# CrispyChillies/Image-Retrieval---Thesis-2026

Measured on AMD Instinct MI355X. Metric: queries/sec (embed+top-10) over 1M x 1024 gallery, higher is better.
Workload: dtype f32 embed (two fp16 MFMA terms); bf16 MFMA candidates + f64 re-rank

## Files before the change

image-retrieval---thesis-2026_amd/_lib.py:

```python
import ctypes
import os

_HERE = os.path.dirname(os.path.abspath(__file__))
LIB_PATH = os.environ.get("MIRX_LIB_PATH", os.path.join(_HERE, "libmirx.so"))

METRIC_IP = 0
METRIC_NEG_L2 = 1
TIER_AUTO = 0
TIER_EXACT_ONLY = 3
OPT_TIERS = 1
OPT_SAMPLE_RANK = 2
OPT_FORCE_TAU = 3
OPT_PROFILE = 4
OPT_RANK_SORT = 5
RANK_SORT_AUTO = 0
RANK_SORT_BITONIC = 1
RANK_SORT_RADIX = 2
MAX_SEARCH_K = 1024
TUNE_CONV1X1_SMALL_MAX_WG = 1
TUNE_CONV3X3_SMALL_MAX_WG = 2
TUNE_CONV1X1_RING = 3
SIMCAM_MAPS_BOTH = 0
SIMCAM_MAPS_RETRIEVED = 1
SIMATT_GROUP = 0
SIMATT_PAIRS = 1
ANOMALY_BAD_SCORE = 1
ANOMALY_BAD_NORM = 2
ANOMALY_BAD_ONE_CLASS = 4
ANOMALY_BAD_EMPTY_CLASS = 8
RESAMPLE_MAX_SIDE = 8192
RESAMPLE_MAX_TAPS = 65
RESAMPLE_MAX_OUT = 1024
RESAMPLE_MAX_BATCH = 65536
RESAMPLE_MAX_LDS = 65536
RESAMPLE_TILE_W, RESAMPLE_TILE_H = 32, 16
RESAMPLE_DESC_WORDS = 8
# ... 9 lines not shown

class SearchStats(ctypes.Structure):
    _fields_ = [(n, ctypes.c_int64) for n in
                ("nq", "tier1_answered", "exact_answered", "candidates", "reranked",
                 "overflowed", "incomplete")]

    def as_dict(self):
        return {n: int(getattr(self, n)) for n, _ in self._fields_}


_vp, _i64, _int = ctypes.c_void_p, ctypes.c_int64, ctypes.c_int
SYMBOLS = {
    "mirx_last_error": (ctypes.c_char_p, []),
    "mirx_version": (_int, []),
    "mirx_set_tuning": (_int, [_int, _i64]),
    "mirx_index_create": (_int, [_int, _int, _int, ctypes.POINTER(_vp)]),
    "mirx_index_destroy": (None, [_vp]),
    "mirx_index_add": (_int, [_vp, _vp, _i64, _vp]),
    "mirx_index_reserve": (_int, [_vp, _i64]),
    "mirx_index_size": (_i64, [_vp]),
    "mirx_index_dim": (_int, [_vp]),
    "mirx_index_set_option": (_int, [_vp, _int, _i64]),
    "mirx_index_get_rows": (_int, [_vp, _i64, _i64, _vp, _vp]),
    "mirx_index_search": (_int, [_vp, _vp, _i64, _int, _vp, _vp, _vp, _vp]),
    "mirx_index_search_f64": (_int, [_vp, _vp, _i64, _int, _vp, _vp, _vp, _vp]),
    "mirx_index_search_begin": (_int, [_vp, _vp, _i64, _int, _vp, _vp, _vp, _vp, _vp]),
    "mirx_index_search_end": (_int, [_vp]),
    "mirx_index_last_stats": (_int, [_vp, _vp, ctypes.POINTER(SearchStats)]),
    "mirx_index_last_timings": (_int, [_vp, ctypes.POINTER(ctypes.c_float)]),
    "mirx_index_rank_all": (_int, [_vp, _vp, _i64, _vp, _vp, _vp, _vp]),
# ... 35 lines not shown
    "mirx_dense_layer_fused": (_int, [_vp, _i64, _i64, _int, _vp, _vp, _vp, _vp, _vp, _vp, _vp, _i64, _int, _vp, ctypes.c_float,
                                      ctypes.c_float, ctypes.c_float, ctypes.c_float, _vp]),
    "mirx_conv3x3_direct_terms_nchw": (_int, [_vp, _vp, _vp, _i64, _int, _vp, _i64, _vp, _vp, _i64, _vp]),
    "mirx_conv3x3_direct_terms_nchw_pool": (_int, [_vp, _vp, _vp, _i64, _int, _vp, _i64, _vp, _vp, _i64, _vp, _vp, _vp, _i64, _vp]),
    "mirx_conv3x3_small_launch": (_int, [_i64, _int]),
    "mirx_conv3x3_winograd_split3_nchw": (_int, [_vp, _vp, _i64, _int, _vp, _i64, _vp]),
    "mirx_conv3x3_direct_split3_nchw": (_int, [_vp, _vp, _i64, _int, _vp, _i64, _vp]),
    "mirx_conv3x3_winograd_nchw": (_int, [_vp, _vp, _i64, _int, _vp, _i64, _vp]),
    "mirx_attention_qkv_f32": (_int, [_vp, _i64, _int, _int, _int, ctypes.c_float, _vp, _vp]),
    "mirx_attention_qkv_f32_split2h": (_int, [_vp, _i64, _int, _int, _int, ctypes.c_float, ctypes.c_float, ctypes.c_float, _vp, _vp]),
    "mirx_attention_qkv_f32_split2h_terms": (_int, [_vp, _i64, _int, _int, _int, ctypes.c_float, ctypes.c_float, ctypes.c_float,
                                                    ctypes.c_float, _vp, _vp]),
    "mirx_attention_qkv_f32_split3": (_int, [_vp, _i64, _int, _int, _int, ctypes.c_float, _vp, _vp]),
    "mirx_l2_normalize": (_int, [_vp, _i64, _int, _vp]),
    "mirx_bn_relu_gap_l2norm": (_int, [_vp, _vp, _vp, _i64, _int, _int, _int, _vp, _vp]),
    "mirx_bn_relu_nchw": (_int, [_vp, _i64, _vp, _vp, _i64, _int, _int, _vp, _vp]),
    "mirx_bn_relu_avgpool2": (_int, [_vp, _i64, _vp, _vp, _i64, _int, _int, _int, _vp, _i64, _vp]),
    "mirx_bn_relu_avgpool2_into": (_int, [_vp, _i64, _vp, _vp, _i64, _int, _int, _int, _vp, _i64, _i64, _vp]),
    "mirx_conv1x1_bn_relu": (_int, [_vp, _i64, _int, _vp, _vp, _vp, _vp, _i64, _int, _int, _int, _vp, _vp]),
    "mirx_dwconv7x7_nchw_to_nhwc": (_int, [_vp, _vp, _vp, _i64, _int, _int, _int, _vp, _vp]),
    "mirx_dwconv7x7_nhwc": (_int, [_vp, _vp, _vp, _i64, _int, _int, _int, _vp, _vp]),
    "mirx_stem_conv7_bn_relu_pool_split3": (_int, [_vp, _vp, _vp, _vp, _i64, _int, _int, _vp, _vp]),
    "mirx_stem_conv7_bn_relu_pool": (_int, [_vp, _vp, _vp, _vp, _i64, _int, _int, _vp, _vp]),
    "mirx_conv_terms": (_int, [_vp, _vp, _vp, _i64, _int, _int, _int, _int, _int, _vp, _vp, _vp, _int, ctypes.c_float,
                               ctypes.c_float, _vp, _vp, _vp, _int, _vp, _vp, _vp, _vp, _vp]),
    "mirx_nchw_to_terms": (_int, [_vp, _i64, _i64, _int, _int, _vp, _vp, _vp, _vp]),
    "mirx_gap_nhwc_l2norm": (_int, [_vp, _i64, _int, _int, _int, _vp, _vp]),
    "mirx_window_attention_split2h": (_int, [_vp, _i64, _int, _int, _int, _int, _int, _vp, _vp, _vp, _vp, ctypes.c_float, _vp]),
    "mirx_swin_postnorm": (_int, [_vp, _vp, _i64, _int, _vp, _vp, ctypes.c_float, _vp, _vp, ctypes.c_float, _vp]),
    "mirx_patch_merge_terms": (_int, [_vp, _i64, _int, _int, _int, ctypes.c_float, _vp, _vp]),
# ... 82 lines not shown
```

image-retrieval---thesis-2026_amd/csrc/k_conv1x1_h2.hip:

```cpp
#include <atomic>

#include "mirx_device.h"
#include "mirx_kernels.h"

namespace mirx {

namespace {

#ifdef MIRX_C1H2_STAMPS
__device__ unsigned long long g_c1_stamps[8192 * 8];
#define C1_STAMP(ACC)                                                 \
    {                                                                 \
        const unsigned long long now_ = __builtin_amdgcn_s_memtime(); \
        ACC += now_ - st_t;                                           \
        st_t = now_;                                                  \
    }
#else
#define C1_STAMP(ACC)
#endif

constexpr int CM = 128;
constexpr int CP = 128;
constexpr int KC = 16;
constexpr int PLANE_A = CM * KC * 2;
// ... 650 lines not shown
#pragma unroll
            for (int mi = 0; mi < 4; ++mi)
#pragma unroll
                for (int r = 0; r < 16; ++r) {
                    const int ch = mi * 32 + (r & 3) + 8 * (r >> 2) + 4 * (lane >> 5);
                    float v = fmaf(acc[mi][ni][r], TABLED ? sOsc[ep_k[ni]][ch] : sOsc[0][ch] * x_inv, sBias[ch]);
                    if (RELU_OUT) v = v < 0.f ? 0.f : v;
                    vmax = range_max(vmax, v);
                    yo[(int64_t)(co0 + ch) * yps] = v;
                }
        }
        if (out_amax) range_publish_lanes(out_amax, (int)bimg, vmax, lane);
    }
}

template <bool PROLOGUE, bool RELU_OUT, bool YTERMS, int NPT, bool TABLED, bool RING>
__global__ __launch_bounds__(256, NPT == 2 ? 2 : 3) void k_conv1x1_h2(C1H2_PARAMS) {
    if constexpr (RING) conv1x1_ring<PROLOGUE, RELU_OUT, YTERMS, TABLED>(C1H2_ARGS);
    else conv1x1_tiled<PROLOGUE, RELU_OUT, YTERMS, NPT, TABLED>(C1H2_ARGS);
}

}

#ifdef MIRX_C1H2_STAMPS
extern "C" int mirx_debug_c1_stamps(unsigned long long *out) {
    return (int)hipMemcpyFromSymbol(out, HIP_SYMBOL(g_c1_stamps), sizeof(g_c1_stamps));
}
#endif

static std::atomic<int> g_small_max_wg{128};
void set_conv1x1_small_max_wg(int v) { g_small_max_wg.store(v < 0 ? 0 : v); }
static int conv1x1_small_max_wg() { return g_small_max_wg.load(std::memory_order_relaxed); }
static std::atomic<int> g_ring{1};
void set_conv1x1_ring(int v) { g_ring.store(v ? 1 : 0); }
static bool conv1x1_ring_enabled() { return g_ring.load(std::memory_order_relaxed) != 0; }

hipError_t launch_conv1x1_h2(const float *x, int64_t xbs, int cin, const float *scale, const float *shift,
                             const uint16_t *w2, const float *oscale, const float *bias, int64_t n, int hw, int cout,
                             int relu_out, float *y, int64_t ybs, const float *in_amax, float in_ks, float in_kb,
                             float *out_amax, float y_ks, float y_kb, float *y_inv_out, int64_t xps, int64_t yps,
                             hipStream_t st) {
    if (n <= 0) return hipSuccess;
    if (cin % KC || cout % CM || !oscale) return hipErrorInvalidValue;
    const bool yterms = y_inv_out != nullptr;
    if (yterms && (cout != CM || !relu_out || !scale)) return hipErrorInvalidValue;
    if (!xps) xps = hw;
    if (!yps) yps = hw;
    if (xps < hw || yps < hw) return hipErrorInvalidValue;
    const int64_t px = n * (int64_t)hw;
    if (px >= ((int64_t)1 << 31) - 2 * CP) return hipErrorInvalidValue;
    if (yterms && px >= ((int64_t)1 << 27)) return hipErrorInvalidValue;
    const bool small_bn_ok = !scale || (cin <= 1024 && ((reinterpret_cast<uintptr_t>(scale) | reinterpret_cast<uintptr_t>(shift)) & 15) == 0);
    if (px * (cout / CM) < (int64_t)CP * conv1x1_small_max_wg() && small_bn_ok)
        return launch_conv1x1_h2_small(x, xbs, cin, scale, shift, w2, oscale, bias, n, hw, cout, relu_out, y, ybs, in_amax,
                                       in_ks, in_kb, out_amax, y_ks, y_kb, y_inv_out, xps, yps, st);
    const int npt = px >= (int64_t)2 * CP * MIRX_C1H2_MIN_WG ? MIRX_C1H2_NPT : 1;
    const bool ring = npt == 2 && conv1x1_ring_enabled() && hw % 4 == 0 && xps % 4 == 0 && xbs % 4 == 0 &&
                      (reinterpret_cast<uintptr_t>(x) & 15) == 0 && (!scale || cin <= RING_BN_MAX_CIN) &&
                      ((int64_t)((RNP - 1) / hw + 2) * xbs + (int64_t)cin * xps) * 4 < ((int64_t)1 << 31);
    const dim3 grid((unsigned)((px + CP * npt - 1) / (CP * npt)), (unsigned)(cout / CM));
    const size_t lds = ring ? (size_t)RING_BN + (scale ? (size_t)cin * 8 : 0) : 2 * (size_t)(2 * PLANE_A + npt * 2 * PLANE_B);
    unsigned *oa = reinterpret_cast<unsigned *>(out_amax);
    const bool tabled = (CP * npt - 1) / hw + 2 <= 8;
#define MIRX_H2K(P, R, T, N, RG)                                                                           \
    {                                                                                                      \
        if (tabled) MIRX_H2KT(P, R, T, N, true, RG) else MIRX_H2KT(P, R, T, N, false, RG)                  \
    }
#define MIRX_H2KT(P, R, T, N, TB, RG)                                                                      \
    {                                                                                                      \
        static std::atomic<unsigned long long> attr_devs{0};       \
        hipError_t e = set_dynamic_lds(k_conv1x1_h2<P, R, T, N, TB, RG>, RG ? RING_BN + 8 * RING_BN_MAX_CIN : 2 * (2 * PLANE_A + N * 2 * PLANE_B), &attr_devs);    \
        if (e != hipSuccess) return e;                                                                 \
        hipLaunchKernelGGL((k_conv1x1_h2<P, R, T, N, TB, RG>), grid, dim3(256), lds, st, x, xbs, cin, scale, shift, w2, oscale, \
                           bias, n, hw, cout, y, ybs, in_amax, in_ks, in_kb, oa, y_ks, y_kb, y_inv_out, xps, yps); \
    }
#define MIRX_H2C(P, R, T)                                                                                  \
    {                                                                                                      \
// ... 17 lines not shown
```

image-retrieval---thesis-2026_amd/csrc/k_prep.hip:

```cpp
#include "mirx_device.h"
#include "mirx_kernels.h"

#include <algorithm>

namespace mirx {

namespace {

__device__ inline double row_sumsq_lane_tree(const float *__restrict__ x, int dim) {
    const int lane = lane_id();
    const int nchunk = (dim + 3) >> 2;
    const bool vec = ((dim & 3) == 0) && ((reinterpret_cast<uintptr_t>(x) & 15) == 0);
    double acc = 0.0;
    for (int c = lane; c < nchunk; c += WAVE) {
        float v[4];
        if (vec) {
            const float4 t = *reinterpret_cast<const float4 *>(x + 4 * c);
            v[0] = t.x; v[1] = t.y; v[2] = t.z; v[3] = t.w;
        } else {
#pragma unroll
            for (int e = 0; e < 4; ++e) v[e] = (4 * c + e < dim) ? x[4 * c + e] : 0.0f;
        }
#pragma unroll
        for (int e = 0; e < 4; ++e) acc = fma((double)v[e], (double)v[e], acc);
// ... 55 lines not shown
}

__global__ __launch_bounds__(256) void k_l2_normalize(float *__restrict__ x, int64_t n, int dim) {
    const int64_t row = (int64_t)blockIdx.x * 4 + (threadIdx.x >> 6);
    if (row >= n) return;
    float *r = x + row * dim;
    const double ss = row_sumsq_lane_tree(r, dim);
    double nrm = sqrt(ss);
    if (nrm < 1e-12) nrm = 1e-12;
    for (int e = lane_id(); e < dim; e += WAVE) r[e] = (float)((double)r[e] / nrm);
}

constexpr int HEAD_THREADS = 1024;
__global__ __launch_bounds__(HEAD_THREADS) void k_head(const float *__restrict__ x,
                                              const float *__restrict__ scale,
                                              const float *__restrict__ shift, int c, int hw,
                                              int normalize, float *__restrict__ y) {
    extern __shared__ __attribute__((aligned(16))) float mean_s[];
    const int64_t b = blockIdx.x;
    const int wave = threadIdx.x >> 6, lane = lane_id();
    const float *xb = x + b * (int64_t)c * hw;
    const float inv = 1.0f / (float)hw;
    constexpr int UC = 8;
    for (int ch0 = wave * UC; ch0 < c; ch0 += (HEAD_THREADS / WAVE) * UC) {
        float acc[UC];
#pragma unroll
        for (int u = 0; u < UC; ++u) {
            const int ch = ch0 + u < c ? ch0 + u : c - 1;
            const float sc = scale ? scale[ch] : 1.0f, sh = shift ? shift[ch] : 0.0f;
            const float *p = xb + (int64_t)ch * hw;
            acc[u] = 0.0f;
            for (int i = lane; i < hw; i += WAVE) {
                const float t = fmaf(p[i], sc, sh);
                acc[u] += t < 0.0f ? 0.0f : t;
            }
        }
#pragma unroll
        for (int u = 0; u < UC; ++u) {
#pragma unroll
            for (int off = 32; off >= 1; off >>= 1) acc[u] += __shfl_xor(acc[u], off, 64);
            if (lane == 0 && ch0 + u < c) mean_s[ch0 + u] = acc[u] * inv;
        }
    }
    const int cpad = (c + 3) & ~3;
    double *nrm_s = reinterpret_cast<double *>(mean_s + cpad);
    for (int i = c + threadIdx.x; i < cpad; i += HEAD_THREADS) mean_s[i] = 0.0f;
    __syncthreads();
    if (normalize) {
        if (wave == 0) {
            const double ss = row_sumsq_lane_tree(mean_s, c);
            double nrm = sqrt(ss);
            if (nrm < 1e-12) nrm = 1e-12;
            if (lane == 0) *nrm_s = nrm;
        }
        __syncthreads();
        const double nrm = *nrm_s;
        for (int i = threadIdx.x; i < c; i += HEAD_THREADS) y[b * c + i] = (float)((double)mean_s[i] / nrm);
    } else {
        for (int i = threadIdx.x; i < c; i += HEAD_THREADS) y[b * c + i] = mean_s[i];
    }
}

__global__ __launch_bounds__(256) void k_bn_relu(const float *__restrict__ x, int64_t xbs,
                                                 const float *__restrict__ scale,
                                                 const float *__restrict__ shift, int c, int hw,
                                                 float *__restrict__ y) {
    const int64_t b = blockIdx.y;
    const int64_t slab = (int64_t)c * hw;
    const float *xb = x + b * xbs;
    float *yb = y + b * slab;
    const float inv_hw = 1.0f / (float)hw;
    for (int64_t e = ((int64_t)blockIdx.x * 256 + threadIdx.x) * 4; e < slab; e += (int64_t)gridDim.x * 1024) {
        const float4 v = *reinterpret_cast<const float4 *>(xb + e);
        int ch = (int)((float)e * inv_hw);
// ... 102 lines not shown

hipError_t launch_prep_queries(const float *q, int64_t nq, int64_t nq_pad, int dim, int dimp,
                               float *q32p, uint16_t *q16, float *qnorm, hipStream_t st) {
    if (nq_pad <= 0) return hipSuccess;
    hipLaunchKernelGGL(k_prep_queries, dim3((unsigned)((nq_pad + 3) / 4)), dim3(256), 0, st, q, nq,
                       nq_pad, dim, dimp, q32p, q16, qnorm);
    return hipGetLastError();
}

hipError_t launch_l2_normalize(float *x, int64_t n, int dim, hipStream_t st) {
    if (n <= 0) return hipSuccess;
    hipLaunchKernelGGL(k_l2_normalize, dim3((unsigned)((n + 3) / 4)), dim3(256), 0, st, x, n, dim);
    return hipGetLastError();
}

hipError_t launch_bn_relu_gap_l2norm(const float *x, const float *scale, const float *shift,
                                     int64_t n, int c, int hw, int normalize, float *y,
                                     hipStream_t st) {
    if (n <= 0) return hipSuccess;
    const size_t lds = (size_t)((c + 3) & ~3) * sizeof(float) + 16;
    hipLaunchKernelGGL(k_head, dim3((unsigned)n), dim3(HEAD_THREADS), lds, st, x, scale, shift, c, hw,
                       normalize, y);
    return hipGetLastError();
}

}
```

image-retrieval---thesis-2026_amd/csrc/mirx_api.hip:

```cpp
#include <algorithm>
#include <cmath>
#include <cstring>
#include <new>
#include <mutex>
#include <vector>

#include "mirx_kernels.h"

namespace mirx {

static thread_local std::string g_err;
void set_error(const std::string &msg) { g_err = msg; }
int fail(int code, const std::string &msg) {
    g_err = msg;
    return code;
}

static inline int64_t round_up(int64_t v, int64_t m) { return (v + m - 1) / m * m; }

struct DevBuf {
    void *p = nullptr;
    size_t bytes = 0;
    hipError_t ensure(size_t need) {
        if (need <= bytes) return hipSuccess;
// ... 490 lines not shown

int mirx_set_tuning(int key, int64_t value) {
    switch (key) {
        case MIRX_TUNE_CONV1X1_SMALL_MAX_WG:
            MIRX_CHECK(value >= 0 && value <= (1 << 20), "set_tuning: conv1x1 small-launch limit out of range");
            set_conv1x1_small_max_wg((int)value);
            return MIRX_OK;
        case MIRX_TUNE_CONV3X3_SMALL_MAX_WG:
            MIRX_CHECK(value >= 0 && value <= (1 << 20), "set_tuning: conv3x3 small-launch limit out of range");
            set_conv3x3_small_max_wg((int)value);
            return MIRX_OK;
        case MIRX_TUNE_CONV1X1_RING:
            MIRX_CHECK(value == 0 || value == 1, "set_tuning: conv1x1 ring switch must be 0 or 1");
            set_conv1x1_ring((int)value);
            return MIRX_OK;
        default:
            return fail(MIRX_EINVAL, "set_tuning: unknown key");
    }
}

int mirx_index_create(int dim, int metric, int device, mirx_index **out) {
    MIRX_CHECK(out, "index_create: out is null");
    *out = nullptr;
    MIRX_CHECK(dim >= 1 && round_up(dim, DIM_ALIGN) <= MAX_DIMP, "index_create: dim out of range");
    MIRX_CHECK(metric == MIRX_METRIC_IP || metric == MIRX_METRIC_NEG_L2, "index_create: unknown metric");
    int ndev = 0;
    MIRX_HIP(hipGetDeviceCount(&ndev));
    MIRX_CHECK(device >= 0 && device < ndev, "index_create: no such device");
    DeviceGuard dg(device);
    if (!dg.ok) return fail(MIRX_EHIP, "index_create: cannot select device");
    mirx_index *ix = new (std::nothrow) mirx_index();
    if (!ix) return fail(MIRX_ENOMEM, "index_create: host allocation failed");
// ... 679 lines not shown

int mirx_l2_normalize(float *x, int64_t n, int dim, void *stream) {
    MIRX_CHECK(x && n >= 0 && dim >= 1, "l2_normalize: bad argument");
    MIRX_HIP(launch_l2_normalize(x, n, dim, reinterpret_cast<hipStream_t>(stream)));
    return MIRX_OK;
}

int mirx_bn_relu_gap_l2norm(const float *x, const float *scale, const float *shift, int64_t n, int c,
                            int hw, int normalize, float *y, void *stream) {
    MIRX_CHECK(x && y && n >= 0 && c >= 1 && c <= 16384 && hw >= 1, "bn_relu_gap_l2norm: bad argument");
    MIRX_HIP(launch_bn_relu_gap_l2norm(x, scale, shift, n, c, hw, normalize, y,
                                       reinterpret_cast<hipStream_t>(stream)));
    return MIRX_OK;
}

int mirx_bn_relu_nchw(const float *x, int64_t x_batch_stride, const float *scale, const float *shift,
                      int64_t n, int c, int hw, float *y, void *stream) {
    MIRX_CHECK(x && scale && shift && y && n >= 0 && c >= 1 && hw >= 1, "bn_relu_nchw: bad argument");
    MIRX_CHECK(((int64_t)c * hw) % 4 == 0 && x_batch_stride % 4 == 0 && x_batch_stride >= (int64_t)c * hw,
               "bn_relu_nchw: c*hw and the batch stride must be multiples of 4");
    MIRX_HIP(launch_bn_relu_nchw(x, x_batch_stride, scale, shift, n, c, hw, y,
                                 reinterpret_cast<hipStream_t>(stream)));
    return MIRX_OK;
}

int mirx_bn_relu_avgpool2(const float *x, int64_t x_batch_stride, const float *scale, const float *shift,
                          int64_t n, int c, int h, int w, float *y, int64_t x_plane_stride, void *stream) {
    MIRX_CHECK(x && scale && shift && y && n >= 0 && c >= 1, "bn_relu_avgpool2: bad argument");
    MIRX_CHECK(h >= 2 && w >= 2 && h % 2 == 0 && w % 2 == 0 && x_batch_stride % 2 == 0,
               "bn_relu_avgpool2: h, w and the batch stride must be even");
// ... 343 lines not shown
```

image-retrieval---thesis-2026_amd/csrc/mirx_kernels.h:

```cpp
#pragma once
#include "mirx_common.h"

namespace mirx {

hipError_t launch_ingest(const float *src, int64_t n, int dim, int dimp, float *g32,
                         uint16_t *g16, float *gbias, unsigned *gnorm_max_bits, int metric,
                         hipStream_t st);
hipError_t launch_prep_queries(const float *q, int64_t nq, int64_t nq_pad, int dim, int dimp,
                               float *q32p, uint16_t *q16, float *qnorm, hipStream_t st);
hipError_t launch_l2_normalize(float *x, int64_t n, int dim, hipStream_t st);
hipError_t launch_bn_relu_gap_l2norm(const float *x, const float *scale, const float *shift,
                                     int64_t n, int c, int hw, int normalize, float *y,
                                     hipStream_t st);
hipError_t launch_bn_relu_nchw(const float *x, int64_t x_batch_stride, const float *scale,
                               const float *shift, int64_t n, int c, int hw, float *y, hipStream_t st);
hipError_t launch_bn_relu_avgpool2(const float *x, int64_t x_batch_stride, const float *scale,
                                   const float *shift, int64_t n, int c, int h, int w, float *y,
                                   int64_t x_plane_stride, hipStream_t st, int64_t y_batch_stride = 0);
hipError_t launch_stem(const float *x, const float *w, const float *scale, const float *shift,
                       int64_t n, int h, int wd, float *y, hipStream_t st);
hipError_t launch_stem_s3(const float *x, const uint16_t *w3, const float *scale, const float *shift, int64_t n, int h,
                          int wd, float *y, int64_t y_bs, float *out_range, hipStream_t st);

hipError_t launch_stem_h2(const float *x, const uint16_t *w2, const float *oscale, const float *scale, const float *shift,
                          int64_t n, int h, int wd, float *y, int64_t y_bs, const float *in_range, float *out_range,
                          hipStream_t st);
hipError_t launch_range_absmax(const float *x, int64_t per_image, int64_t n, float *row, hipStream_t st);
hipError_t launch_stem_h2_u8(const uint8_t *x, const float *mean, const float *stdv, const uint16_t *w2, const float *oscale,
// ... 73 lines not shown
hipError_t launch_resample(const void *blob_dev, int64_t b, int s, int out_f32, const float *mean3, const float *std3, void *out,
                           int64_t lds, hipStream_t st);

hipError_t launch_conv1x1_s3(const float *x, int64_t xbs, int cin, const float *scale, const float *shift,
                             const uint16_t *w3, const float *bias, int64_t n, int hw, int cout, int relu_out,
                             float *y, int64_t ybs, hipStream_t st);

hipError_t launch_conv1x1_h2(const float *x, int64_t xbs, int cin, const float *scale, const float *shift,
                             const uint16_t *w2, const float *oscale, const float *bias, int64_t n, int hw, int cout,
                             int relu_out, float *y, int64_t ybs, const float *in_amax, float in_ks, float in_kb,
                             float *out_amax, float y_ks, float y_kb, float *y_inv_out, int64_t xps, int64_t yps,
                             hipStream_t st);

void set_conv1x1_small_max_wg(int v);
void set_conv1x1_ring(int v);
hipError_t launch_conv1x1_h2_small(const float *x, int64_t xbs, int cin, const float *scale, const float *shift,
                                   const uint16_t *w2, const float *oscale, const float *bias, int64_t n, int hw, int cout,
                                   int relu_out, float *y, int64_t ybs, const float *in_amax, float in_ks, float in_kb,
                                   float *out_amax, float y_ks, float y_kb, float *y_inv_out, int64_t xps, int64_t yps,
                                   hipStream_t st);

hipError_t launch_linear_h2(const float *x, int64_t m, int k, const uint16_t *w2, const float *bias, int n, int act,
                            const float *res, const float *gamma, float x_scale, float out_scale, float *y,
                            int tokens_per_image, const float *xb_dev, hipStream_t st, bool rows_out = false,
                            float *sq_out = nullptr);
hipError_t launch_grn_norm_partials(const float *part, int tpi, int64_t n_img, int c, float *gx, hipStream_t st);

hipError_t launch_linear_s3(const float *x, int64_t m, int k, const uint16_t *w3, const float *bias, int n, int act,
                            const float *res, const float *gamma, float *y, int tokens_per_image, hipStream_t st);

// ... 140 lines not shown
```

include/mirx.h:

```cpp
#ifndef MIRX_H
#define MIRX_H

#include <stdint.h>

#ifdef __cplusplus
extern "C" {
#endif

#define MIRX_VERSION 305

#define MIRX_OK 0
#define MIRX_EINVAL (-1)
#define MIRX_ENOMEM (-2)
#define MIRX_EHIP (-3)
#define MIRX_ESTATE (-4)

#define MIRX_METRIC_IP 0
#define MIRX_METRIC_NEG_L2 1

#define MIRX_TIER_AUTO 0
#define MIRX_TIER_EXACT_ONLY 3

#define MIRX_OPT_TIERS 1
#define MIRX_OPT_SAMPLE_RANK 2
// ... 18 lines not shown
    int64_t nq;
    int64_t tier1_answered;
    int64_t exact_answered;
    int64_t candidates;
    int64_t reranked;
    int64_t overflowed;
    int64_t incomplete;
} mirx_search_stats;

const char *mirx_last_error(void);
int mirx_version(void);

#define MIRX_TUNE_CONV1X1_SMALL_MAX_WG 1
#define MIRX_TUNE_CONV3X3_SMALL_MAX_WG 2
#define MIRX_TUNE_CONV1X1_RING 3
int mirx_set_tuning(int key, int64_t value);

int mirx_index_create(int dim, int metric, int device, mirx_index **out);
void mirx_index_destroy(mirx_index *ix);

int mirx_index_add(mirx_index *ix, const float *rows, int64_t n, const int64_t *ids_or_null);
int mirx_index_reserve(mirx_index *ix, int64_t capacity_rows);
int64_t mirx_index_size(const mirx_index *ix);
int mirx_index_dim(const mirx_index *ix);
int mirx_index_set_option(mirx_index *ix, int option, int64_t value);

int mirx_index_get_rows(const mirx_index *ix, int64_t first, int64_t n, float *out_rows,
                        int64_t *out_ids_or_null);

int mirx_index_search(mirx_index *ix, const float *q, int64_t nq, int k,
                      const int64_t *exclude_ids_or_null, float *out_scores, int64_t *out_ids,
// ... 128 lines not shown
                                   float scale, float qk_bound, float v_bound, float *out, void *stream);
int mirx_attention_qkv_f32_split2h_terms(const float *qkv, int64_t batch, int n_tokens, int heads, int head_dim, float scale,
                                         float qk_bound, float v_bound, float out_scale, void *out_terms, void *stream);

int mirx_rank_metrics(const int64_t *ranks, int64_t nq, int64_t n, int64_t row_stride,
                      const int64_t *gallery_labels, int64_t n_labels, const int64_t *query_labels,
                      const int64_t *query_ids_or_null, int drop_self, int rel_kind,
                      double jaccard_threshold, int ap_kind, const int32_t *kappas, int nk,
                      double *out_ap, int64_t *out_cnt, int64_t *out_nrel, int64_t *out_maxpos,
                      void *stream);

int mirx_l2_normalize(float *x, int64_t n, int dim, void *stream);

int mirx_bn_relu_gap_l2norm(const float *x, const float *scale, const float *shift, int64_t n,
                            int c, int hw, int normalize, float *y, void *stream);

int mirx_bn_relu_nchw(const float *x, int64_t x_batch_stride, const float *scale, const float *shift,
                      int64_t n, int c, int hw, float *y, void *stream);

int mirx_bn_relu_avgpool2(const float *x, int64_t x_batch_stride, const float *scale,
                          const float *shift, int64_t n, int c, int h, int w, float *y, int64_t x_plane_stride,
                          void *stream);
int mirx_bn_relu_avgpool2_into(const float *x, int64_t x_batch_stride, const float *scale, const float *shift,
                               int64_t n, int c, int h, int w, float *y, int64_t y_batch_stride, int64_t x_plane_stride,
                               void *stream);

int mirx_stem_conv7_bn_relu_pool(const float *x, const float *w, const float *scale,
                                 const float *shift, int64_t n, int h, int wd, float *y,
                                 void *stream);

// ... 214 lines not shown
```

Baseline: 43070.

## Add wide 256-channel conv1x1 kernel and run-staged GAP head kernel

Adds a conv1x1 variant in which each workgroup computes 256 output channels over 128 pixels, with buffer-to-LDS DMA into a three-slot ring so each input tile is reused across twice as many channels. It is used by default for large no-BN-prologue launches. It also adds a head kernel that stages contiguous runs of small spatial planes in LDS with float4 loads before the BN-ReLU-GAP-L2 reduction, plus tuning switches and launch counters. In exchange, the wide kernel carries a larger accumulator count and more LDS per block, which may reduce occupancy.

```diff
diff --git a/image-retrieval---thesis-2026_amd/_lib.py b/image-retrieval---thesis-2026_amd/_lib.py
--- a/image-retrieval---thesis-2026_amd/_lib.py
+++ b/image-retrieval---thesis-2026_amd/_lib.py
@@ -20,6 +20,9 @@
 TUNE_CONV1X1_SMALL_MAX_WG = 1
 TUNE_CONV3X3_SMALL_MAX_WG = 2
 TUNE_CONV1X1_RING = 3
+TUNE_CONV1X1_WIDE = 4
+TUNE_HEAD_RUNS = 5
+TUNE_CONV1X1_LARGE_MIN_WG = 6
 SIMCAM_MAPS_BOTH = 0
 SIMCAM_MAPS_RETRIEVED = 1
 SIMATT_GROUP = 0
@@ -59,6 +62,7 @@
     "mirx_last_error": (ctypes.c_char_p, []),
     "mirx_version": (_int, []),
     "mirx_set_tuning": (_int, [_int, _i64]),
+    "mirx_launch_count": (_i64, [_int]),
     "mirx_index_create": (_int, [_int, _int, _int, ctypes.POINTER(_vp)]),
     "mirx_index_destroy": (None, [_vp]),
     "mirx_index_add": (_int, [_vp, _vp, _i64, _vp]),
@@ -124,6 +128,7 @@
     "mirx_attention_qkv_f32_split3": (_int, [_vp, _i64, _int, _int, _int, ctypes.c_float, _vp, _vp]),
     "mirx_l2_normalize": (_int, [_vp, _i64, _int, _vp]),
     "mirx_bn_relu_gap_l2norm": (_int, [_vp, _vp, _vp, _i64, _int, _int, _int, _vp, _vp]),
+    "mirx_bn_relu_gap_l2norm_strided": (_int, [_vp, _i64, _vp, _vp, _i64, _int, _int, _int, _vp, _vp]),
     "mirx_bn_relu_nchw": (_int, [_vp, _i64, _vp, _vp, _i64, _int, _int, _vp, _vp]),
     "mirx_bn_relu_avgpool2": (_int, [_vp, _i64, _vp, _vp, _i64, _int, _int, _int, _vp, _i64, _vp]),
     "mirx_bn_relu_avgpool2_into": (_int, [_vp, _i64, _vp, _vp, _i64, _int, _int, _int, _vp, _i64, _i64, _vp]),
diff --git a/image-retrieval---thesis-2026_amd/csrc/k_conv1x1_h2.hip b/image-retrieval---thesis-2026_amd/csrc/k_conv1x1_h2.hip
--- a/image-retrieval---thesis-2026_amd/csrc/k_conv1x1_h2.hip
+++ b/image-retrieval---thesis-2026_amd/csrc/k_conv1x1_h2.hip
@@ -688,6 +688,182 @@
     }
 }
 
+constexpr int WSLOT_W = 2 * 2 * PLANE_A;
+constexpr int WSLOT = WSLOT_W + KC * CP * 4;
+constexpr int WIDE_LDS = RSLOTS * WSLOT;
+
+template <bool RELU_OUT, bool TABLED, bool DW>
+__device__ __forceinline__ void conv1x1_wide(C1H2_PARAMS) {
+    extern __shared__ __attribute__((aligned(16))) char sm[];
+    constexpr int KIMG = 8;
+    constexpr int WCM = 2 * CM;
+    constexpr int PIECES = 4 + (DW ? 8 : 2);
+    const int wave = __builtin_amdgcn_readfirstlane(threadIdx.x >> 6), lane = threadIdx.x & 63;
+    const int tid = threadIdx.x;
+    const int64_t total = n * (int64_t)hw;
+    const int64_t p0 = (int64_t)blockIdx.x * CP;
+    const int co0 = blockIdx.y * WCM;
+    const int nk = cin / KC;
+    auto image_bound = [&](int64_t img) { return fmaf(in_ks, in_amax ? in_amax[img] : 0.f, in_kb); };
+    const unsigned img_first = (unsigned)p0 / (unsigned)hw;
+    const unsigned p_last = (unsigned)(p0 + CP - 1 < total ? p0 + CP - 1 : total - 1);
+
+    const __amdgpu_buffer_rsrc_t wrsrc = __builtin_amdgcn_make_buffer_rsrc(
+        (void *)(w2 + ((int64_t)(2 * blockIdx.y) * nk) * (2 * CM * KC)), 0, 2 * nk * (2 * CM * KC * 2), 0x00020000);
+    const int w_voff = (lane >> 1) * 32 + (((lane & 1) ^ ((lane >> 4) & 1)) << 4);
+    const __amdgpu_buffer_rsrc_t xrsrc =
+        __builtin_amdgcn_make_buffer_rsrc((void *)(x + (int64_t)img_first * xbs), 0, 0x7fffffff, 0x00020000);
+    const int xps4 = (int)xps * 4;
+    auto pixel_voff = [&](unsigned pp) {
+        if (pp >= (unsigned)total) return 0;
+        const unsigned pimg = pp / (unsigned)hw;
+        return (int)(((int64_t)(pimg - img_first) * xbs + (pp - pimg * (unsigned)hw)) * 4);
+    };
+    int x_voff[2];
+    if (DW) {
+        x_voff[0] = pixel_voff((unsigned)p0 + lane);
+        x_voff[1] = pixel_voff((unsigned)p0 + 64u + lane);
+    } else {
+        x_voff[0] = pixel_voff((unsigned)p0 + 4u * (lane & 31)) + (lane >> 5) * xps4;
+        x_voff[1] = 0;
+    }
+    auto dma = [&](int kt, int slot) {
+        char *sb = sm + slot * WSLOT;
+#pragma unroll
+        for (int i = 0; i < 4; ++i) {
+            const int piece = wave + 4 * i;
+            __builtin_amdgcn_raw_ptr_buffer_load_lds(wrsrc, LDS_PTR(sb + piece * 1024), 16, w_voff,
+                                                     ((piece >> 3) * nk + kt) * (2 * CM * KC * 2) + (piece & 7) * 1024, 0, 0);
+        }
+        if (DW) {
+#pragma unroll
+            for (int i = 0; i < 8; ++i) {
+                const int c = 4 * wave + (i >> 1), h = i & 1;
+                __builtin_amdgcn_raw_ptr_buffer_load_lds(xrsrc, LDS_PTR(sb + WSLOT_W + c * (CP * 4) + h * 256), 4, x_voff[h],
+                                                         (kt * KC + c) * xps4, 0, 0);
+            }
+        } else {
+#pragma unroll
+            for (int i = 0; i < 2; ++i) {
+                const int pc = 2 * wave + i;
+                __builtin_amdgcn_raw_ptr_buffer_load_lds(xrsrc, LDS_PTR(sb + WSLOT_W + pc * 1024), 16, x_voff[0],
+                                                         (kt * KC + 2 * pc) * xps4, 0, 0);
+            }
+        }
+    };
+
+    const float t_bias = bias ? bias[co0 + tid] : 0.f;
+    const float t_osc = oscale[co0 + tid];
+    const unsigned nimg = p_last / (unsigned)hw - img_first + 1;
+    float ib[KIMG];
+#pragma unroll
+    for (int k = 0; k < KIMG; ++k) ib[k] = TABLED && (unsigned)k < nimg ? image_bound(img_first + k) : 0.f;
+    unsigned col_img;
+    {
+        unsigned pp = (unsigned)(p0 + 32 * wave + (lane & 31));
+        if (pp >= (unsigned)total) pp = (unsigned)total - 1u;
+        col_img = pp / (unsigned)hw;
+    }
+    const float col_bound = image_bound(col_img);
+    __builtin_amdgcn_sched_barrier(0);
+    dma(0, 0);
+    if (nk > 1) dma(1, 1);
+    __builtin_amdgcn_sched_barrier(0);
+    float x_scale, ep_xinv;
+    range_scales(col_bound, x_scale, ep_xinv);
+    const int ep_k = TABLED ? (int)(col_img - img_first) : 0;
+    if (TABLED) ep_xinv = 1.f;
+
+    const int kg = lane >> 5;
+    int fa[4];
+#pragma unroll
+    for (int mi = 0; mi < 4; ++mi) {
+        const int ra_ = mi * 32 + (lane & 31);
+        fa[mi] = ra_ * 32 + ((kg ^ ((ra_ >> 3) & 1)) << 4);
+    }
+    const int fb = WSLOT_W + 8 * kg * (CP * 4) + (32 * wave + (lane & 31)) * 4;
+
+    f32x16 acc[8];
+#pragma unroll
+    for (int mi = 0; mi < 8; ++mi)
+#pragma unroll
+        for (int r = 0; r < 16; ++r) acc[mi][r] = 0.f;
+
+    int slot = 0;
+    for (int kt = 0; kt < nk; ++kt) {
+        if (kt + 1 < nk) asm volatile("s_waitcnt vmcnt(%0)" ::"n"(PIECES) : "memory");
+        else asm volatile("s_waitcnt vmcnt(0)" ::: "memory");
+        asm volatile("s_waitcnt lgkmcnt(0)\n\ts_barrier" ::: "memory");
+        if (kt + 2 < nk) dma(kt + 2, slot == 0 ? 2 : slot - 1);
+        __builtin_amdgcn_sched_barrier(0);
+        const char *sb = sm + slot * WSLOT;
+        u32x4 ph, pl;
+#pragma unroll
+        for (int j = 0; j < 4; ++j) {
+            const float v0 = *reinterpret_cast<const float *>(sb + fb + (2 * j) * (CP * 4));
+            const float v1 = *reinterpret_cast<const float *>(sb + fb + (2 * j + 1) * (CP * 4));
+            unsigned th, tl;
+            split2h_pair(v0 * x_scale, v1 * x_scale, th, tl);
+            ph[j] = th;
+            pl[j] = tl;
+        }
+        const f16x8 b0 = __builtin_bit_cast(f16x8, ph), b1 = __builtin_bit_cast(f16x8, pl);
+#pragma unroll
+        for (int mi = 0; mi < 8; ++mi) {
+            const f16x8 a0 = *reinterpret_cast<const f16x8 *>(sb + (mi >> 2) * (2 * PLANE_A) + fa[mi & 3]);
+            const f16x8 a1 = *reinterpret_cast<const f16x8 *>(sb + (mi >> 2) * (2 * PLANE_A) + fa[mi & 3] + PLANE_A);
+            f32x16 c = acc[mi];
+            c = __builtin_amdgcn_mfma_f32_32x32x16_f16(a1, b0, c, 0, 0, 0);
+            c = __builtin_amdgcn_mfma_f32_32x32x16_f16(a0, b1, c, 0, 0, 0);
+            c = __builtin_amdgcn_mfma_f32_32x32x16_f16(a0, b0, c, 0, 0, 0);
+            acc[mi] = c;
+        }
+        slot = slot == RSLOTS - 1 ? 0 : slot + 1;
+    }
+
+    float *sBias = reinterpret_cast<float *>(sm + (nk % RSLOTS) * WSLOT);
+    float(*sOsc)[WCM] = reinterpret_cast<float(*)[WCM]>(sBias + WCM);
+    sBias[tid] = t_bias;
+    sOsc[0][tid] = t_osc;
+    if (TABLED) {
+#pragma unroll
+        for (int k = 0; k < KIMG; ++k) {
+            if ((unsigned)k < nimg) {
+                float xs_, xi_;
+                range_scales(ib[k], xs_, xi_);
+                sOsc[k][tid] = t_osc * xi_;
+            }
+        }
+    }
+    asm volatile("s_waitcnt lgkmcnt(0)\n\ts_barrier" ::: "memory");
+
+    unsigned pp = (unsigned)(p0 + 32 * wave + (lane & 31));
+    const bool live = pp < (unsigned)total;
+    if (!live) pp = (unsigned)total - 1u;
+    const unsigned ubimg = pp / (unsigned)hw;
+    const int64_t bimg = ubimg, off = pp - ubimg * (unsigned)hw;
+    float vmax = 0.f;
+    float *yo = y + bimg * ybs + off;
+    if (live) {
+#pragma unroll
+        for (int mi = 0; mi < 8; ++mi)
+#pragma unroll
+            for (int r = 0; r < 16; ++r) {
+                const int ch = mi * 32 + (r & 3) + 8 * (r >> 2) + 4 * (lane >> 5);
+                float v = fmaf(acc[mi][r], TABLED ? sOsc[ep_k][ch] : sOsc[0][ch] * ep_xinv, sBias[ch]);
+                if (RELU_OUT) v = v < 0.f ? 0.f : v;
+                vmax = range_max(vmax, v);
+                yo[(int64_t)(co0 + ch) * yps] = v;
+            }
+    }
+    if (out_amax) range_publish_lanes(out_amax, (int)bimg, vmax, lane);
+}
+
+template <bool RELU_OUT, bool TABLED, bool DW>
+__global__ __launch_bounds__(256, 2) void k_conv1x1_h2w(C1H2_PARAMS) {
+    conv1x1_wide<RELU_OUT, TABLED, DW>(C1H2_ARGS);
+}
+
 template <bool PROLOGUE, bool RELU_OUT, bool YTERMS, int NPT, bool TABLED, bool RING>
 __global__ __launch_bounds__(256, NPT == 2 ? 2 : 3) void k_conv1x1_h2(C1H2_PARAMS) {
     if constexpr (RING) conv1x1_ring<PROLOGUE, RELU_OUT, YTERMS, TABLED>(C1H2_ARGS);
@@ -708,6 +884,12 @@
 static std::atomic<int> g_ring{1};
 void set_conv1x1_ring(int v) { g_ring.store(v ? 1 : 0); }
 static bool conv1x1_ring_enabled() { return g_ring.load(std::memory_order_relaxed) != 0; }
+static std::atomic<int> g_wide{1};
+static std::atomic<long long> g_wide_launches{0};
+void set_conv1x1_wide(int v) { g_wide.store(v ? 1 : 0); }
+long long conv1x1_wide_launches() { return g_wide_launches.load(std::memory_order_relaxed); }
+static std::atomic<int> g_large_min_wg{MIRX_C1H2_MIN_WG};
+void set_conv1x1_large_min_wg(int v) { g_large_min_wg.store(v < 1 ? 1 : v); }
 
 hipError_t launch_conv1x1_h2(const float *x, int64_t xbs, int cin, const float *scale, const float *shift,
                              const uint16_t *w2, const float *oscale, const float *bias, int64_t n, int hw, int cout,
@@ -728,13 +910,40 @@
     if (px * (cout / CM) < (int64_t)CP * conv1x1_small_max_wg() && small_bn_ok)
         return launch_conv1x1_h2_small(x, xbs, cin, scale, shift, w2, oscale, bias, n, hw, cout, relu_out, y, ybs, in_amax,
                                        in_ks, in_kb, out_amax, y_ks, y_kb, y_inv_out, xps, yps, st);
-    const int npt = px >= (int64_t)2 * CP * MIRX_C1H2_MIN_WG ? MIRX_C1H2_NPT : 1;
+    const int npt = px >= (int64_t)2 * CP * g_large_min_wg.load(std::memory_order_relaxed) ? MIRX_C1H2_NPT : 1;
+    unsigned *oa = reinterpret_cast<unsigned *>(out_amax);
+    if (npt == 2 && !scale && !yterms && cout % (2 * CM) == 0 && g_wide.load(std::memory_order_relaxed) &&
+        ((int64_t)((CP - 1) / hw + 2) * xbs + (int64_t)cin * xps) * 4 < ((int64_t)1 << 31)) {
+        const bool dw = !(hw % 4 == 0 && xps % 4 == 0 && xbs % 4 == 0 && (reinterpret_cast<uintptr_t>(x) & 15) == 0);
+        const bool wtabled = (CP - 1) / hw + 2 <= 8;
+        const dim3 wgrid((unsigned)((px + CP - 1) / CP), (unsigned)(cout / (2 * CM)));
+#define MIRX_H2W(R, TB, D)                                                                                 \
+    {                                                                                                      \
+        static std::atomic<unsigned long long> attr_devs{0};                                               \
+        hipError_t e = set_dynamic_lds(k_conv1x1_h2w<R, TB, D>, WIDE_LDS, &attr_devs);                     \
+        if (e != hipSuccess) return e;                                                                     \
+        hipLaunchKernelGGL((k_conv1x1_h2w<R, TB, D>), wgrid, dim3(256), WIDE_LDS, st, x, xbs, cin, scale, shift, w2, oscale, \
+                           bias, n, hw, cout, y, ybs, in_amax, in_ks, in_kb, oa, y_ks, y_kb, y_inv_out, xps, yps); \
+    }
+#define MIRX_H2W_T(R, TB)                                                                                  \
+    {                                                                                                      \
+        if (dw) MIRX_H2W(R, TB, true) else MIRX_H2W(R, TB, false)                                          \
+    }
+        if (relu_out) {
+            if (wtabled) MIRX_H2W_T(true, true) else MIRX_H2W_T(true, false)
+        } else {
+            if (wtabled) MIRX_H2W_T(false, true) else MIRX_H2W_T(false, false)
+        }
+#undef MIRX_H2W
+#undef MIRX_H2W_T
+        g_wide_launches.fetch_add(1, std::memory_order_relaxed);
+        return hipGetLastError();
+    }
     const bool ring = npt == 2 && conv1x1_ring_enabled() && hw % 4 == 0 && xps % 4 == 0 && xbs % 4 == 0 &&
                       (reinterpret_cast<uintptr_t>(x) & 15) == 0 && (!scale || cin <= RING_BN_MAX_CIN) &&
                       ((int64_t)((RNP - 1) / hw + 2) * xbs + (int64_t)cin * xps) * 4 < ((int64_t)1 << 31);
     const dim3 grid((unsigned)((px + CP * npt - 1) / (CP * npt)), (unsigned)(cout / CM));
     const size_t lds = ring ? (size_t)RING_BN + (scale ? (size_t)cin * 8 : 0) : 2 * (size_t)(2 * PLANE_A + npt * 2 * PLANE_B);
-    unsigned *oa = reinterpret_cast<unsigned *>(out_amax);
     const bool tabled = (CP * npt - 1) / hw + 2 <= 8;
 #define MIRX_H2K(P, R, T, N, RG)                                                                           \
     {                                                                                                      \
diff --git a/image-retrieval---thesis-2026_amd/csrc/k_prep.hip b/image-retrieval---thesis-2026_amd/csrc/k_prep.hip
--- a/image-retrieval---thesis-2026_amd/csrc/k_prep.hip
+++ b/image-retrieval---thesis-2026_amd/csrc/k_prep.hip
@@ -2,6 +2,7 @@
 #include "mirx_kernels.h"
 
 #include <algorithm>
+#include <atomic>
 
 namespace mirx {
 
@@ -93,12 +94,12 @@
 constexpr int HEAD_THREADS = 1024;
 __global__ __launch_bounds__(HEAD_THREADS) void k_head(const float *__restrict__ x,
                                               const float *__restrict__ scale,
-                                              const float *__restrict__ shift, int c, int hw,
+                                              const float *__restrict__ shift, int c, int hw, int64_t xps,
                                               int normalize, float *__restrict__ y) {
     extern __shared__ __attribute__((aligned(16))) float mean_s[];
     const int64_t b = blockIdx.x;
     const int wave = threadIdx.x >> 6, lane = lane_id();
-    const float *xb = x + b * (int64_t)c * hw;
+    const float *xb = x + b * (int64_t)c * xps;
     const float inv = 1.0f / (float)hw;
     constexpr int UC = 8;
     for (int ch0 = wave * UC; ch0 < c; ch0 += (HEAD_THREADS / WAVE) * UC) {
@@ -107,7 +108,7 @@
         for (int u = 0; u < UC; ++u) {
             const int ch = ch0 + u < c ? ch0 + u : c - 1;
             const float sc = scale ? scale[ch] : 1.0f, sh = shift ? shift[ch] : 0.0f;
-            const float *p = xb + (int64_t)ch * hw;
+            const float *p = xb + (int64_t)ch * xps;
             acc[u] = 0.0f;
             for (int i = lane; i < hw; i += WAVE) {
                 const float t = fmaf(p[i], sc, sh);
@@ -137,6 +138,82 @@
         for (int i = threadIdx.x; i < c; i += HEAD_THREADS) y[b * c + i] = (float)((double)mean_s[i] / nrm);
     } else {
         for (int i = threadIdx.x; i < c; i += HEAD_THREADS) y[b * c + i] = mean_s[i];
+    }
+}
+
+constexpr int HEADR_CH = HEAD_THREADS / 4;
+constexpr int HEADR_NL = 4;
+__global__ __launch_bounds__(HEAD_THREADS) void k_head_runs(const float *__restrict__ x, const float *__restrict__ scale,
+                                                            const float *__restrict__ shift, int c, int hw, int xps,
+                                                            int normalize, float *__restrict__ y) {
+    extern __shared__ __attribute__((aligned(16))) float run_s[];
+    float *mean_s = run_s + HEADR_CH * xps;
+    const int64_t b = blockIdx.x;
+    const int tid = threadIdx.x, wave = tid >> 6, lane = lane_id();
+    const float4 *xb = reinterpret_cast<const float4 *>(x + b * (int64_t)c * xps);
+    const float inv = 1.0f / (float)hw;
+    const int chl = tid >> 2, q = tid & 3;
+    float4 r[HEADR_NL];
+    auto load = [&](int ch0) {
+        const int nch = c - ch0 < HEADR_CH ? c - ch0 : HEADR_CH;
+        const int nf4 = nch * xps >> 2;
+        const float4 *src = xb + ((int64_t)ch0 * xps >> 2);
+#pragma unroll
+        for (int i = 0; i < HEADR_NL; ++i) {
+            const int e = tid + HEAD_THREADS * i;
+            r[i] = e < nf4 ? src[e] : make_float4(0.f, 0.f, 0.f, 0.f);
+        }
+    };
+    load(0);
+    for (int ch0 = 0; ch0 < c; ch0 += HEADR_CH) {
+        const int nch = c - ch0 < HEADR_CH ? c - ch0 : HEADR_CH;
+        const int nf4 = nch * xps >> 2;
+#pragma unroll
+        for (int i = 0; i < HEADR_NL; ++i) {
+            const int e = tid + HEAD_THREADS * i;
+            if (e < nf4) reinterpret_cast<float4 *>(run_s)[e] = r[i];
+        }
+        __syncthreads();
+        if (ch0 + HEADR_CH < c) load(ch0 + HEADR_CH);
+        const int ch = ch0 + chl < c ? ch0 + chl : c - 1;
+        const float sc = scale ? scale[ch] : 1.0f, sh = shift ? shift[ch] : 0.0f;
+        const float *p = run_s + (ch - ch0) * xps;
+        float v[16];
+#pragma unroll
+        for (int m = 0; m < 16; ++m) {
+            const int j = q + 4 * m;
+            v[m] = 0.0f;
+            if (j < hw) {
+                const float t = fmaf(p[j], sc, sh);
+                v[m] += t < 0.0f ? 0.0f : t;
+            }
+        }
+#pragma unroll
+        for (int w = 8; w >= 1; w >>= 1)
+#pragma unroll
+            for (int m = 0; m < w; ++m) v[m] += v[m + w];
+        float s = v[0];
+        s += __shfl_xor(s, 2, 64);
+        s += __shfl_xor(s, 1, 64);
+        if (q == 0 && ch0 + chl < c) mean_s[ch0 + chl] = s * inv;
+        __syncthreads();
+    }
+    const int cpad = (c + 3) & ~3;
+    double *nrm_s = reinterpret_cast<double *>(mean_s + cpad);
+    for (int i = c + tid; i < cpad; i += HEAD_THREADS) mean_s[i] = 0.0f;
+    __syncthreads();
+    if (normalize) {
+        if (wave == 0) {
+            const double ss = row_sumsq_lane_tree(mean_s, c);
+            double nrm = sqrt(ss);
+            if (nrm < 1e-12) nrm = 1e-12;
+            if (lane == 0) *nrm_s = nrm;
+        }
+        __syncthreads();
+        const double nrm = *nrm_s;
+        for (int i = tid; i < c; i += HEAD_THREADS) y[b * c + i] = (float)((double)mean_s[i] / nrm);
+    } else {
+        for (int i = tid; i < c; i += HEAD_THREADS) y[b * c + i] = mean_s[i];
     }
 }
 
@@ -269,12 +346,31 @@
     return hipGetLastError();
 }
 
+static std::atomic<int> g_head_runs{1};
+static std::atomic<long long> g_head_runs_launches{0};
+void set_head_runs(int v) { g_head_runs.store(v ? 1 : 0); }
+long long head_runs_launches() { return g_head_runs_launches.load(std::memory_order_relaxed); }
+
 hipError_t launch_bn_relu_gap_l2norm(const float *x, const float *scale, const float *shift,
                                      int64_t n, int c, int hw, int normalize, float *y,
-                                     hipStream_t st) {
-    if (n <= 0) return hipSuccess;
+                                     hipStream_t st, int64_t x_plane_stride) {
+    if (n <= 0) return hipSuccess;
+    if (!x_plane_stride) x_plane_stride = hw;
+    if (x_plane_stride < hw) return hipErrorInvalidValue;
     const size_t lds = (size_t)((c + 3) & ~3) * sizeof(float) + 16;
-    hipLaunchKernelGGL(k_head, dim3((unsigned)n), dim3(HEAD_THREADS), lds, st, x, scale, shift, c, hw,
+    const size_t lds_runs = lds + (size_t)HEADR_CH * x_plane_stride * sizeof(float);
+    constexpr size_t HEADR_MAX_LDS = 80 * 1024;
+    if (g_head_runs.load(std::memory_order_relaxed) && x_plane_stride <= 16 * HEADR_NL && ((int64_t)c * x_plane_stride & 3) == 0 &&
+        (reinterpret_cast<uintptr_t>(x) & 15) == 0 && lds_runs <= HEADR_MAX_LDS) {
+        static std::atomic<unsigned long long> attr_devs{0};
+        const hipError_t e = set_dynamic_lds(k_head_runs, HEADR_MAX_LDS, &attr_devs);
+        if (e != hipSuccess) return e;
+        hipLaunchKernelGGL(k_head_runs, dim3((unsigned)n), dim3(HEAD_THREADS), lds_runs, st, x, scale, shift, c, hw,
+                           (int)x_plane_stride, normalize, y);
+        g_head_runs_launches.fetch_add(1, std::memory_order_relaxed);
+        return hipGetLastError();
+    }
+    hipLaunchKernelGGL(k_head, dim3((unsigned)n), dim3(HEAD_THREADS), lds, st, x, scale, shift, c, hw, x_plane_stride,
                        normalize, y);
     return hipGetLastError();
 }
diff --git a/image-retrieval---thesis-2026_amd/csrc/mirx_api.hip b/image-retrieval---thesis-2026_amd/csrc/mirx_api.hip
--- a/image-retrieval---thesis-2026_amd/csrc/mirx_api.hip
+++ b/image-retrieval---thesis-2026_amd/csrc/mirx_api.hip
@@ -528,8 +528,28 @@
             MIRX_CHECK(value == 0 || value == 1, "set_tuning: conv1x1 ring switch must be 0 or 1");
             set_conv1x1_ring((int)value);
             return MIRX_OK;
+        case MIRX_TUNE_CONV1X1_WIDE:
+            MIRX_CHECK(value == 0 || value == 1, "set_tuning: conv1x1 wide switch must be 0 or 1");
+            set_conv1x1_wide((int)value);
+            return MIRX_OK;
+        case MIRX_TUNE_CONV1X1_LARGE_MIN_WG:
+            MIRX_CHECK(value >= 1 && value <= (1 << 20), "set_tuning: conv1x1 large-launch limit out of range");
+            set_conv1x1_large_min_wg((int)value);
+            return MIRX_OK;
+        case MIRX_TUNE_HEAD_RUNS:
+            MIRX_CHECK(value == 0 || value == 1, "set_tuning: head runs switch must be 0 or 1");
+            set_head_runs((int)value);
+            return MIRX_OK;
         default:
             return fail(MIRX_EINVAL, "set_tuning: unknown key");
+    }
+}
+
+int64_t mirx_launch_count(int key) {
+    switch (key) {
+        case MIRX_TUNE_CONV1X1_WIDE: return conv1x1_wide_launches();
+        case MIRX_TUNE_HEAD_RUNS: return head_runs_launches();
+        default: fail(MIRX_EINVAL, "launch_count: this key has no counter"); return -1;
     }
 }
 
@@ -1239,6 +1259,14 @@
     return MIRX_OK;
 }
 
+int mirx_bn_relu_gap_l2norm_strided(const float *x, int64_t x_plane_stride, const float *scale, const float *shift, int64_t n,
+                                    int c, int hw, int normalize, float *y, void *stream) {
+    MIRX_CHECK(x && y && n >= 0 && c >= 1 && c <= 16384 && hw >= 1 && x_plane_stride >= hw, "bn_relu_gap_l2norm_strided: bad argument");
+    MIRX_HIP(launch_bn_relu_gap_l2norm(x, scale, shift, n, c, hw, normalize, y, reinterpret_cast<hipStream_t>(stream),
+                                       x_plane_stride));
+    return MIRX_OK;
+}
+
 int mirx_bn_relu_nchw(const float *x, int64_t x_batch_stride, const float *scale, const float *shift,
                       int64_t n, int c, int hw, float *y, void *stream) {
     MIRX_CHECK(x && scale && shift && y && n >= 0 && c >= 1 && hw >= 1, "bn_relu_nchw: bad argument");
diff --git a/image-retrieval---thesis-2026_amd/csrc/mirx_kernels.h b/image-retrieval---thesis-2026_amd/csrc/mirx_kernels.h
--- a/image-retrieval---thesis-2026_amd/csrc/mirx_kernels.h
+++ b/image-retrieval---thesis-2026_amd/csrc/mirx_kernels.h
@@ -11,7 +11,9 @@
 hipError_t launch_l2_normalize(float *x, int64_t n, int dim, hipStream_t st);
 hipError_t launch_bn_relu_gap_l2norm(const float *x, const float *scale, const float *shift,
                                      int64_t n, int c, int hw, int normalize, float *y,
-                                     hipStream_t st);
+                                     hipStream_t st, int64_t x_plane_stride = 0);
+void set_head_runs(int v);
+long long head_runs_launches();
 hipError_t launch_bn_relu_nchw(const float *x, int64_t x_batch_stride, const float *scale,
                                const float *shift, int64_t n, int c, int hw, float *y, hipStream_t st);
 hipError_t launch_bn_relu_avgpool2(const float *x, int64_t x_batch_stride, const float *scale,
@@ -115,6 +117,9 @@
 
 void set_conv1x1_small_max_wg(int v);
 void set_conv1x1_ring(int v);
+void set_conv1x1_wide(int v);
+long long conv1x1_wide_launches();
+void set_conv1x1_large_min_wg(int v);
 hipError_t launch_conv1x1_h2_small(const float *x, int64_t xbs, int cin, const float *scale, const float *shift,
                                    const uint16_t *w2, const float *oscale, const float *bias, int64_t n, int hw, int cout,
                                    int relu_out, float *y, int64_t ybs, const float *in_amax, float in_ks, float in_kb,
diff --git a/include/mirx.h b/include/mirx.h
--- a/include/mirx.h
+++ b/include/mirx.h
@@ -56,7 +56,11 @@
 #define MIRX_TUNE_CONV1X1_SMALL_MAX_WG 1
 #define MIRX_TUNE_CONV3X3_SMALL_MAX_WG 2
 #define MIRX_TUNE_CONV1X1_RING 3
+#define MIRX_TUNE_CONV1X1_WIDE 4
+#define MIRX_TUNE_HEAD_RUNS 5
+#define MIRX_TUNE_CONV1X1_LARGE_MIN_WG 6
 int mirx_set_tuning(int key, int64_t value);
+int64_t mirx_launch_count(int key);
 
 int mirx_index_create(int dim, int metric, int device, mirx_index **out);
 void mirx_index_destroy(mirx_index *ix);
@@ -215,6 +219,8 @@
 
 int mirx_bn_relu_gap_l2norm(const float *x, const float *scale, const float *shift, int64_t n,
                             int c, int hw, int normalize, float *y, void *stream);
+int mirx_bn_relu_gap_l2norm_strided(const float *x, int64_t x_plane_stride, const float *scale, const float *shift, int64_t n,
+                                    int c, int hw, int normalize, float *y, void *stream);
 
 int mirx_bn_relu_nchw(const float *x, int64_t x_batch_stride, const float *scale, const float *shift,
                       int64_t n, int c, int hw, float *y, void *stream);
```

Result: faster. 43530 (median of 6 runs) (+1.1%).
